# zouyuoz/SVS-UNet-PyTorch

Hardware: AMD Instinct MI355X
Metric: spectrogram-tiles/sec (512x128) U-Net fwd+bwd (L1 train step incl. Adam) (higher is better)
Workload: dtype f32; 1 GPU; train.py L1-loss step, 512x128 tiles, batch 64 per GPU; global_batch=64, parallelism=dp1, mode=train

## Files before the change

### include/svs_hip.h

```cpp
#ifndef SVS_HIP_H
#define SVS_HIP_H

#include <stddef.h>
#include <stdint.h>

typedef struct ihipStream_t* hipStream_t;

#ifdef __cplusplus
extern "C" {
#endif

#define SVS_OK 0
#define SVS_ERR_INVALID (-1)
#define SVS_ERR_WORKSPACE (-2)
#define SVS_ABI_VERSION 1

int svs_version(void);
const char* svs_last_error_string(void);
int svs_tuning_set(const char* name, long value);

int svs_fill_uniform(float* out, int64_t n, uint32_t seed, uint64_t offset, float scale, float shift,
                     hipStream_t stream);
int svs_fill_tiles(float* mix, float* voc, int B, int H, int W, int64_t first_tile, hipStream_t stream);
int svs_crop_tiles(const float* mix_songs, const float* voc_songs, const int64_t* offset, const int32_t* frames,
// ... 49 lines not shown
int svs_bn_act_apply(const float* raw, int64_t ldr, int64_t P, int C, int64_t pixels_per_sample,
                     const float* gamma, const float* beta, const float* save_mean, const float* save_invstd,
                     float slope, const float* drop, float* y, int64_t ldy, hipStream_t stream);
int svs_bn_bwd(const float* dy, int64_t lddy, const float* raw, int64_t ldr, int64_t P, int C,
               int64_t pixels_per_sample, const float* gamma, const float* beta,
               const float* save_mean, const float* save_invstd, float slope, const float* drop,
               float* d_raw, float* dgamma, float* dbeta, void* ws, size_t ws_bytes, hipStream_t stream);

size_t svs_l1_mask_loss_workspace_bytes(int64_t n);
int svs_l1_mask_loss_fwd_bwd(const float* mask, const float* mix, const float* voc, int64_t n, float loss_scale,
                             float* d_logit, float* loss, void* ws, size_t ws_bytes, hipStream_t stream);

int svs_adam_step(float* p, const float* g, float* m, float* v, int64_t n, double lr, double beta1, double beta2,
                  double eps, int step, float grad_scale, hipStream_t stream);

int svs_apply_mask(const float* mix, const float* mask, float* out, int64_t n, int invert, hipStream_t stream);

#define SVS_UNET_NUM_PARAMS 46
#define SVS_UNET_NUM_BN 11
int64_t svs_unet_param_offset(int tensor_index);
int64_t svs_unet_buffer_offset(int bn_index, int which );

size_t svs_unet_prepared_bytes(void);
int svs_unet_prepare_eval(const float* params, const float* bn_buffers, void* prepared, hipStream_t stream);
size_t svs_unet_eval_workspace_bytes(int B, int H, int W);
int svs_unet_forward_eval(const void* prepared, const float* mix, float* mask, int B, int H, int W,
                          void* ws, size_t ws_bytes, hipStream_t stream);

size_t svs_unet_train_workspace_bytes(int B, int H, int W);
int svs_unet_train_fwd_bwd(const float* params, float* grads, float* bn_buffers, int64_t* num_batches_tracked,
                           const float* mix, const float* voc, const float* drop, int B, int H, int W,
                           float loss_scale, float* mask , float* loss,
                           void* ws, size_t ws_bytes, hipStream_t stream);
int svs_unet_train_forward(const float* params, float* bn_buffers, int64_t* num_batches_tracked,
                           const float* mix, const float* drop, int B, int H, int W, float* mask,
                           void* ws, size_t ws_bytes, hipStream_t stream);
int svs_unet_train_backward(const float* params, float* grads, const float* mix, const float* mask,
                            const float* d_mask, const float* drop, int B, int H, int W,
                            void* ws, size_t ws_bytes, hipStream_t stream);
int svs_unet_train_fwd_loss(const float* params, float* bn_buffers, int64_t* num_batches_tracked, const float* mix,
                            const float* voc, const float* drop, int B, int H, int W, float loss_scale,
                            float* mask , float* loss, void* ws, size_t ws_bytes, hipStream_t stream);
int svs_unet_train_bwd_part(const float* params, float* grads, const float* mix, const float* drop, int B, int H, int W,
                            int part, void* ws, size_t ws_bytes, hipStream_t stream);
int svs_unet_train_bwd_sync(hipStream_t consumer);
size_t svs_unet_train_mr_workspace_bytes(int B, int W, int hop);
int svs_unet_train_fwd_loss_mr(const float* params, float* bn_buffers, int64_t* num_batches_tracked, const float* mix,
                               const float* voc, const float* mix_phase, const float* voc_phase, const float* drop, int B, int H,
                               int W, int hop, float alpha_l1, float alpha_mr, float* mask, float* losses, void* ws, size_t ws_bytes,
                               void* mr_ws, size_t mr_ws_bytes, hipStream_t stream);
int64_t svs_unet_ws_offset(const char* name, int B, int H, int W, int training);

size_t svs_unet_prepared_bf16_bytes(void);
int svs_unet_prepare_eval_bf16(const void* prepared_f32, void* prepared_bf16, hipStream_t stream);
size_t svs_unet_eval_bf16_workspace_bytes(int B, int H, int W);
int svs_unet_forward_eval_bf16(const void* prepared_bf16, const float* mix, float* mask, int B, int H, int W, void* ws,
                               size_t ws_bytes, hipStream_t stream);

int svs_stft_frames(int64_t n_samples, int hop);
int svs_stft_fwd(const float* y, int64_t n_samples, int n_fft, int hop, float* mag, float* phase,
                 hipStream_t stream);
size_t svs_istft_workspace_bytes(int n_fft, int hop, int frames);
int svs_istft(const float* mag, const float* phase, int phase_is_angle, int n_fft, int hop, int frames,
              float* y, void* ws, size_t ws_bytes, hipStream_t stream);
int svs_stft_tiles(const float* y, int64_t n_samples, int channels, int n_fft, int hop, float* mag, int64_t chan_stride,
                   int seg, int rows, int first_bin, int frames_alloc, float* phase, int phase_mode,
// ... 50 lines not shown
```

### svs_unet_pytorch_amd/_lib.py

```python
from __future__ import annotations

import ctypes as C
import os
import re

HERE = os.path.dirname(os.path.abspath(__file__))
LIB_PATH = os.environ.get("SVS_LIB_PATH") or os.path.join(HERE, "libsvs_hip.so")
HEADER_PATH = os.path.join(os.path.dirname(HERE), "include", "svs_hip.h")

_lib = None

P = C.c_void_p
I = C.c_int
L = C.c_int64
F = C.c_float
D = C.c_double
Z = C.c_size_t
U32 = C.c_uint32
U64 = C.c_uint64

_SIGS = {
    "svs_version": (I, []),
    "svs_last_error_string": (C.c_char_p, []),
    "svs_tuning_set": (I, [C.c_char_p, C.c_long]),
    "svs_fill_uniform": (I, [P, L, U32, U64, F, F, P]),
    "svs_fill_tiles": (I, [P, P, I, I, I, L, P]),
    "svs_crop_tiles": (I, [P, P, P, P, P, P, I, I, I, P, P, P]),
    "svs_phase_angle": (I, [P, P, L, P]),
    "svs_dropout_mask": (I, [P, I, I, I, U32, I, I, P]),
    "svs_dropout_masks_all": (I, [P, I, U32, I, I, P]),
    "svs_pack_weight_gather": (I, [P, P, I, I, P]),
    "svs_pack_weight_parity": (I, [P, P, I, I, P]),
    "svs_bn_fold": (I, [P, P, P, P, P, F, P, P, I, P]),
    "svs_enc_block_workspace_bytes": (Z, [I, I, I, I, I]),
    "svs_enc_block_fwd": (I, [P, L, I, I, I, I, P, P, P, P, F, P, L, I, I, P, Z, P]),
    "svs_dec_block_workspace_bytes": (Z, [I, I, I, I, I, I, I]),
    "svs_dec_block_fwd": (I, [P, L, I, I, I, I, P, P, P, P, F, P, L, I, I, I, I, P, Z, P]),
    "svs_out_block_fwd": (I, [P, L, I, I, I, I, P, P, P, I, I, I, P]),
    "svs_enc_block_bwd_data": (I, [P, L, I, I, I, I, P, P, L, I, I, I, I, P, Z, P]),
    "svs_dec_block_bwd_data": (I, [P, L, I, I, I, I, P, P, L, I, I, I, I, P, Z, P]),
    "svs_block_bwd_weight_workspace_bytes": (Z, [I, I, I, I, I]),
    "svs_enc_block_bwd_weight": (I, [P, L, I, I, I, I, P, L, I, I, I, P, P, P, Z, P]),
    "svs_dec_block_bwd_weight": (I, [P, L, I, I, I, I, P, L, I, I, I, P, P, P, Z, P]),
    "svs_describe_plan": (I, [I, I, I, I, I, I, I, I, C.c_char_p, Z]),
    "svs_bn_workspace_bytes": (Z, [L, I]),
    "svs_bn_stats": (I, [P, L, L, I, P, Z, P]),
    "svs_bn_finalize": (I, [P, L, I, F, F, P, P, P, P, P, P]),
    "svs_bn_act_apply": (I, [P, L, L, I, L, P, P, P, P, F, P, P, L, P]),
    "svs_bn_bwd": (I, [P, L, P, L, L, I, L, P, P, P, P, F, P, P, P, P, P, Z, P]),
    "svs_l1_mask_loss_workspace_bytes": (Z, [L]),
    "svs_l1_mask_loss_fwd_bwd": (I, [P, P, P, L, F, P, P, P, Z, P]),
    "svs_adam_step": (I, [P, P, P, P, L, D, D, D, D, I, F, P]),
    "svs_apply_mask": (I, [P, P, P, L, I, P]),
    "svs_unet_param_offset": (L, [I]),
    "svs_unet_buffer_offset": (L, [I, I]),
    "svs_unet_prepared_bytes": (Z, []),
    "svs_unet_prepare_eval": (I, [P, P, P, P]),
    "svs_unet_eval_workspace_bytes": (Z, [I, I, I]),
    "svs_unet_forward_eval": (I, [P, P, P, I, I, I, P, Z, P]),
    "svs_unet_prepared_bf16_bytes": (Z, []),
    "svs_unet_prepare_eval_bf16": (I, [P, P, P]),
    "svs_unet_eval_bf16_workspace_bytes": (Z, [I, I, I]),
    "svs_unet_forward_eval_bf16": (I, [P, P, P, I, I, I, P, Z, P]),
    "svs_unet_train_workspace_bytes": (Z, [I, I, I]),
    "svs_unet_train_fwd_bwd": (I, [P, P, P, P, P, P, P, I, I, I, F, P, P, P, Z, P]),
    "svs_unet_train_forward": (I, [P, P, P, P, P, I, I, I, P, P, Z, P]),
    "svs_unet_train_backward": (I, [P, P, P, P, P, P, I, I, I, P, Z, P]),
    "svs_unet_train_fwd_loss": (I, [P, P, P, P, P, P, I, I, I, F, P, P, P, Z, P]),
    "svs_unet_train_bwd_part": (I, [P, P, P, P, I, I, I, I, P, Z, P]),
    "svs_unet_train_bwd_sync": (I, [P]),
    "svs_unet_train_mr_workspace_bytes": (Z, [I, I, I]),
    "svs_unet_train_fwd_loss_mr": (I, [P, P, P, P, P, P, P, P, I, I, I, I, F, F, P, P, P, Z, P, Z, P]),
    "svs_unet_ws_offset": (L, [C.c_char_p, I, I, I, I]),
    "svs_stft_frames": (I, [L, I]),
    "svs_stft_fwd": (I, [P, L, I, I, P, P, P]),
    "svs_istft_workspace_bytes": (Z, [I, I, I]),
    "svs_istft": (I, [P, P, I, I, I, I, P, P, Z, P]),
    "svs_stft_tiles": (I, [P, L, I, I, I, P, L, I, I, I, I, P, I, P, P]),
    "svs_stft_groups": (I, [I]),
    "svs_istft_tiles": (I, [P, L, I, I, I, P, I, P, I, I, I, I, I, P, P, P]),
    "svs_istft_groups": (I, [I, I, I]),
    "svs_transpose_c64": (I, [P, P, I, I, P]),
    "svs_istft_bwd_mask": (I, [P, P, P, P, P, F, I, I, I, I, P]),
    "svs_mrstft_workspace_bytes": (Z, [I, L]),
    "svs_mrstft_loss_fwd_bwd": (I, [P, P, I, L, F, P, P, P, Z, P]),
    "svs_absmax": (I, [P, L, P, P, Z, P]),
    "svs_max": (I, [P, L, P, P]),
    "svs_scale_by_inv": (I, [P, L, P, F, P]),
    "svs_bss_corr_workspace_bytes": (Z, [L, I, P]),
    "svs_bss_corr": (I, [P, L, I, L, P, I, P, P, Z, P]),
    "svs_bss_solve_workspace_bytes": (Z, [I, I, I]),
    "svs_bss_solve": (I, [P, I, I, P, P, I, P, P, P, Z, P]),
    "svs_bss_corr_windows_workspace_bytes": (Z, [L, L, I, P]),
    "svs_bss_corr_windows": (I, [P, L, I, L, L, L, L, P, I, P, L, P, Z, P]),
    "svs_bss_solve_batched_workspace_bytes": (Z, [L, I, I, I]),
    "svs_bss_solve_batched": (I, [P, L, I, I, P, P, I, P, P, P, Z, P]),
    "svs_resample_out_len": (L, [L, I, I]),
    "svs_resample_table_bytes": (Z, [I, I, I]),
# ... 50 lines not shown
```

### svs_unet_pytorch_amd/csrc/elementwise.hip

```cpp
#include "unet_desc.h"

static inline int red_blocks(long P, int C) {
  long nb = (P * C) / 4096;
  if (nb > 1024) nb = 1024;
  if (nb < 1) nb = 1;
  return (int)nb;
}

struct RedPlan { int sw, nslab, lp, rows; long ppr; };
static RedPlan red_plan(long P, int C) {
  RedPlan r;
  r.sw = C < 32 ? C : 32;
  r.nslab = C / r.sw;
  r.lp = r.sw / 4;
  long nb = (P * C) / 4096;
  if (nb > 512) nb = 512;
  long rows = nb / r.nslab;
  if (rows < 1) rows = 1;
  r.ppr = (P + rows - 1) / rows;
  r.rows = (int)((P + r.ppr - 1) / r.ppr);
  return r;
}
static inline int red_rows(long P, int C) { return red_plan(P, C).rows; }

// ... 593 lines not shown
}
extern "C" int svs_scale_by_inv(float* x, int64_t n, const float* denom, float numer, hipStream_t stream) {
  SVS_REQUIRE(x && denom && n > 0, "svs_scale_by_inv: null pointer");
  hipLaunchKernelGGL(scale_by_inv_kernel, dim3(grid_for(n)), dim3(256), 0, stream, x, (long)n, denom, numer);
  SVS_CHECK_LAUNCH("scale_by_inv");
  return SVS_OK;
}

__global__ __launch_bounds__(256) void adam_kernel(float* __restrict__ p, const float* __restrict__ g, float* __restrict__ m,
                                                   float* __restrict__ v, long n, float b1, float b2, float omb1,
                                                   float omb2, float eps, float step_size, float bc2_sqrt, float gscale) {
  for (long i = (long)blockIdx.x * 256 + threadIdx.x; i < n; i += (long)gridDim.x * 256) {
    const float gi = g[i] * gscale;
    const float mi = m[i] * b1 + omb1 * gi;
    const float vi = v[i] * b2 + omb2 * gi * gi;
    m[i] = mi;
    v[i] = vi;
    const float denom = sqrtf(vi) / bc2_sqrt + eps;
    p[i] -= step_size * (mi / denom);
  }
}
extern "C" int svs_adam_step(float* p, const float* g, float* m, float* v, int64_t n, double lr, double beta1, double beta2,
                             double eps, int step, float grad_scale, hipStream_t stream) {
  SVS_REQUIRE(p && g && m && v && n > 0 && step >= 1, "svs_adam_step: bad arguments");
  const double bc1 = 1.0 - pow(beta1, step);
  const double bc2 = 1.0 - pow(beta2, step);
  hipLaunchKernelGGL(adam_kernel, dim3(grid_for(n)), dim3(256), 0, stream, p, g, m, v, (long)n, (float)beta1,
                     (float)beta2, (float)(1.0 - beta1), (float)(1.0 - beta2), (float)eps, (float)(lr / bc1), (float)sqrt(bc2),
                     grad_scale);
  SVS_CHECK_LAUNCH("adam");
  return SVS_OK;
}

__global__ __launch_bounds__(256) void apply_mask_kernel(const float* __restrict__ mix, const float* __restrict__ mask,
                                                         float* __restrict__ out, long n, int invert) {
  for (long i = (long)blockIdx.x * 256 + threadIdx.x; i < n; i += (long)gridDim.x * 256) {
    float m = mask[i];
    if (invert) m = 1.f - m;
    out[i] = mix[i] * m;
  }
}
extern "C" int svs_apply_mask(const float* mix, const float* mask, float* out, int64_t n, int invert, hipStream_t stream) {
  SVS_REQUIRE(mix && mask && out && n > 0, "svs_apply_mask: null pointer");
  hipLaunchKernelGGL(apply_mask_kernel, dim3(grid_for(n)), dim3(256), 0, stream, mix, mask, out, (long)n, invert);
  SVS_CHECK_LAUNCH("apply_mask");
  return SVS_OK;
}

__global__ __launch_bounds__(256) void pack_gather_kernel(const float* __restrict__ w, float* __restrict__ wp, int N, int C) {
  const long total = (long)N * C * 25;
  for (long o = (long)blockIdx.x * 256 + threadIdx.x; o < total; o += (long)gridDim.x * 256) {
    const int c = (int)(o % C);
    const long r = o / C;
    const int tap = (int)(r % 25);
    const long n = r / 25;
    wp[o] = w[(n * C + c) * 25 + tap];
  }
}
extern "C" int svs_pack_weight_gather(const float* w, float* wp, int N, int C, hipStream_t stream) {
  SVS_REQUIRE(w && wp && N > 0 && C > 0, "svs_pack_weight_gather: bad arguments");
  hipLaunchKernelGGL(pack_gather_kernel, dim3(grid_for((long)N * C * 25)), dim3(256), 0, stream, w, wp, N, C);
  SVS_CHECK_LAUNCH("pack_gather");
  return SVS_OK;
}

__global__ __launch_bounds__(256) void pack_parity_kernel(const float* __restrict__ w, float* __restrict__ wp, int C, int N) {
// ... 44 lines not shown
    for (int e = threadIdx.x; e < tot; e += 256) {
      const int c = e / 25, tap = e - c * 25;
      tile[e] = jb.w[((long)c * N + n) * 25 + tap];
    }
    __syncthreads();
    const long NC = (long)N * C;
#pragma unroll
    for (int par = 0; par < 4; ++par) {
      const int ph = par >> 1, pw = par & 1, ntw = 3 - pw, ntaps = (3 - ph) * ntw;
      const int poff = (par == 0) ? 0 : (par == 1) ? 9 : (par == 2) ? 15 : 21;
      float* dst = jb.wp + poff * NC + (long)n * ntaps * C;
      for (int e = threadIdx.x; e < ntaps * C; e += 256) {
        const int t2 = lc >= 0 ? e >> lc : e / C, c = e - t2 * C;
        const int th = t2 / ntw, tw = t2 - th * ntw;
        dst[e] = tile[c * 25 + (ph + 2 * th) * 5 + pw + 2 * tw];
      }
    }
  }
}

int svs_pack_all_run(SvsPackJobs& jobs, hipStream_t stream) {
  int blocks = 0;
  for (int i = 0; i < jobs.n; ++i) {
    SVS_REQUIRE(jobs.j[i].C <= 512 && jobs.j[i].w && jobs.j[i].wp, "svs_pack_all: bad job %d", i);
    jobs.j[i].first_block = blocks;
    blocks += jobs.j[i].N;
  }
  if (!blocks) return SVS_OK;
  hipLaunchKernelGGL(pack_all_kernel, dim3(blocks), dim3(256), 0, stream, jobs);
  SVS_CHECK_LAUNCH("pack_all");
  return SVS_OK;
}

__global__ void bn_fold_kernel(const float* gamma, const float* beta, const float* rm, const float* rv, const float* bias,
                               float eps, float* scale, float* shift, int C) {
  const int c = blockIdx.x * blockDim.x + threadIdx.x;
  if (c >= C) return;
  const float s = gamma[c] / sqrtf(rv[c] + eps);
  scale[c] = s;
  shift[c] = beta[c] + ((bias ? bias[c] : 0.f) - rm[c]) * s;
}
extern "C" int svs_bn_fold(const float* gamma, const float* beta, const float* running_mean, const float* running_var,
                           const float* conv_bias, float eps, float* scale, float* shift, int C, hipStream_t stream) {
  SVS_REQUIRE(gamma && beta && running_mean && running_var && scale && shift && C > 0, "svs_bn_fold: bad arguments");
  hipLaunchKernelGGL(bn_fold_kernel, dim3((C + 63) / 64), dim3(64), 0, stream, gamma, beta, running_mean, running_var,
                     conv_bias, eps, scale, shift, C);
  SVS_CHECK_LAUNCH("bn_fold");
  return SVS_OK;
}

__global__ __launch_bounds__(256) void fill_uniform_kernel(float* out, long n, uint32_t seed, uint64_t offset, float scale, float shift) {
  for (long i = (long)blockIdx.x * 256 + threadIdx.x; i < n; i += (long)gridDim.x * 256)
    out[i] = (float)(svs_u32(seed, offset + (uint64_t)i) >> 8) * 5.9604644775390625e-08f * scale + shift;
}
extern "C" int svs_fill_uniform(float* out, int64_t n, uint32_t seed, uint64_t offset, float scale, float shift, hipStream_t stream) {
  SVS_REQUIRE(out && n > 0, "svs_fill_uniform: bad arguments");
  hipLaunchKernelGGL(fill_uniform_kernel, dim3(grid_for(n)), dim3(256), 0, stream, out, (long)n, seed, offset, scale, shift);
  SVS_CHECK_LAUNCH("fill_uniform");
  return SVS_OK;
}

__global__ __launch_bounds__(256) void fill_tiles_kernel(float* mix, float* voc, long per, long total, long first_tile) {
  for (long i = (long)blockIdx.x * 256 + threadIdx.x; i < total; i += (long)gridDim.x * 256) {
    const long b = i / per;
    const uint64_t ctr = (uint64_t)(i - b * per) + ((uint64_t)(first_tile + b) << 32);
    const float m = (float)(svs_u32(0u, ctr) >> 8) * 5.9604644775390625e-08f;
// ... 87 lines not shown
```

### svs_unet_pytorch_amd/csrc/internal.h

```cpp
#pragma once
#include "common.h"

enum { SVS_MODE_GATHER = 0, SVS_MODE_PARITY = 1 };

int svs_conv_gemm_run(int mode, const float* x, long ldx, int B, int H, int W, int C, const float* wp,
                      const float* bias, const float* scale, const float* shift, float slope, float* y, long ldy,
                      int Ho, int Wo, int N, int accumulate, void* ws, size_t ws_bytes, hipStream_t stream,
                      const char* who, float* stats = nullptr, int stats_cap = 0, int* stats_nblk = nullptr);
int svs_bn_finalize_run(const void* partial, int nblk, long P, int C, float eps, float momentum, float* running_mean,
                        float* running_var, long long* nbt, float* save_mean, float* save_invstd, hipStream_t stream);
int svs_bn_fin_act_apply_run(const void* partial, int rows, const float* raw, long ldr, long P, int C, long pixels_per_sample,
                             const float* gamma, const float* beta, float eps, float momentum, float* running_mean,
                             float* running_var, long long* nbt, float* save_mean, float* save_invstd, float slope,
                             const float* drop, float* y, long ldy, hipStream_t stream);
struct SvsSumJobs { int njobs; const float* partial[12]; int nblk[12]; int C[12]; float* out[12]; };
int svs_channel_sum_finalize_multi_run(const SvsSumJobs& jobs, hipStream_t stream);
size_t svs_bn_partial_floats(long P, int C);
int svs_bn_partial_rows(long P, int C);
size_t svs_conv_gemm_workspace(int mode, int B, int H, int W, int C, int Ho, int Wo, int N);

int svs_wgrad_gemm_run(const float* s, long lds, int B, int Hs, int Ws, int Cs, const float* l, long ldl, int Hl,
                       int Wl, int Cl, float* dw, void* ws, size_t ws_bytes, hipStream_t stream, const char* who);
size_t svs_wgrad_gemm_workspace(int B, int Hs, int Ws, int Cs, int Cl);

int svs_conv_c1_run(const float* x, int B, int H, int W, const float* w, const float* bias, const float* scale,
                    const float* shift, float slope, float* y, long ldy, int N, int accumulate, hipStream_t stream,
                    const char* who, long half = 0);
int svs_deconv_to1_run(const float* x, long ldx, int B, int H, int W, int C, const float* w, const float* bias,
                       float* y, int Ho, int Wo, int apply_sigmoid, hipStream_t stream, const char* who, long half = 0);
int svs_wgrad_c1_run(const float* s, long lds, int B, int Hs, int Ws, int Cs, const float* l, int Hl, int Wl,
                     float* dw, void* ws, size_t ws_bytes, hipStream_t stream, const char* who, long half = 0);
size_t svs_wgrad_c1_workspace(int B, int Hs, int Ws, int Cs);

int svs_channel_sum_run(const float* x, long ldx, long P, int C, float* out, void* ws, size_t ws_bytes, hipStream_t stream);
int svs_sum_run(const float* x, long n, float* out, void* ws, size_t ws_bytes, hipStream_t stream);
int svs_sigmoid_bwd_run(const float* mask, const float* dmask, long n, float* d_logit, hipStream_t stream);

int svs_reduce_slabs_run(const float* slab, int nslab, int per, int groups, long n, float* out, hipStream_t stream);

struct SvsPackJob { const float* w; float* wp; int N, C, kind, first_block; };
struct SvsPackJobs { SvsPackJob j[20]; int n; };
int svs_pack_all_run(SvsPackJobs& jobs, hipStream_t stream);

int svs_bn_bwd_run(const float* dy, long lddy, const float* raw, long ldr, long P, int C, long pixels_per_sample,
                   const float* gamma, const float* beta, const float* save_mean, const float* save_invstd, float slope,
                   const float* drop, float* d_raw, float* dgamma, float* dbeta, float* dbias, void* ws, size_t ws_bytes,
                   hipStream_t stream, float* dbias_partial = nullptr, SvsSumJobs* defer = nullptr);

int svs_fft_twiddles(int n, hipStream_t stream, const float2** out);

int svs_conv_gemm_describe(int mode, int B, int H, int W, int C, int Ho, int Wo, int N, long ldx, char* buf, size_t n);
int svs_wgrad_gemm_describe(int B, int Hs, int Ws, int Cs, int Cl, char* buf, size_t n);
```

### svs_unet_pytorch_amd/csrc/net.hip

```cpp
#include <math.h>
#include <algorithm>
#include <atomic>
#include <mutex>
#include <stdarg.h>
#include <stdlib.h>
#include <string.h>

#include "unet_desc.h"

static thread_local char g_err[512] = "";
void svs_set_error(const char* fmt, ...) {
  va_list ap;
  va_start(ap, fmt);
  vsnprintf(g_err, sizeof(g_err), fmt, ap);
  va_end(ap);
}
extern "C" const char* svs_last_error_string(void) { return g_err; }

static const char* const TUNE_NAMES[SVS_TUNE_COUNT] = {
    "CONV_CFG", "CONV_KSPLIT", "CONV_WINDOW", "CONV_SKIP", "SKIP_REDUCE", "WGRAD_CFG", "WGRAD_KSPLIT", "WGRAD_SKIP",
    "WGRAD_WINDOW", "TRAIN_UNFUSED", "TRAIN_ONE_STREAM", "MFMA_SPLIT", "CONV_C1_TILED", "BF16_CFG", "BF16_KSPLIT", "BN_INLINE",
    "CONV_GWINDOW"};
static std::atomic<long> g_tune[SVS_TUNE_COUNT];
static std::once_flag g_tune_once;
// ... 293 lines not shown
  }
  return g_side[dev];
}

extern "C" size_t svs_unet_train_workspace_bytes(int B, int H, int W) {
  Geo g;
  if (make_geo(B, H, W, g)) return 0;
  return train_layout(g, nullptr).total;
}

struct WsName { const char* stem; int first, count; float* const* p; };
static int64_t ws_find(const WsName* tab, size_t n, const char* name, const char* base) {
  for (size_t i = 0; i < n; ++i) {
    const size_t len = strlen(tab[i].stem);
    if (strncmp(name, tab[i].stem, len)) continue;
    if (!tab[i].count) {
      if (!name[len]) return (const char*)*tab[i].p - base;
      continue;
    }
    char* end;
    const long idx = strtol(name + len, &end, 10) - tab[i].first;
    if (end != name + len && !*end && idx >= 0 && idx < tab[i].count) return (const char*)tab[i].p[idx] - base;
  }
  return -1;
}
extern "C" int64_t svs_unet_ws_offset(const char* name, int B, int H, int W, int training) {
  Geo g;
  if (!name || make_geo(B, H, W, g)) return -1;
  char* const base = (char*)256;
  if (training) {
    const TrainWs t = train_layout(g, base);
    const WsName tab[] = {{"cat", 1, 5, t.cat + 1}, {"c6", 0, 0, &t.c6},         {"raw_e", 1, 6, t.raw},  {"raw_d", 1, 5, t.raw + 6},
                          {"dcat", 1, 5, t.dcat + 1}, {"dc6", 0, 0, &t.dc6},     {"d_logit", 0, 0, &t.d_logit}, {"mask", 0, 0, &t.mask},
                          {"mean", 0, 11, t.mean},  {"invstd", 0, 11, t.invstd}};
    return ws_find(tab, sizeof(tab) / sizeof(tab[0]), name, base);
  }
  const EvalWs e = eval_layout(g, base);
  const WsName tab[] = {{"cat", 1, 5, e.cat + 1}, {"c6", 0, 0, &e.c6}};
  return ws_find(tab, sizeof(tab) / sizeof(tab[0]), name, base);
}

struct TrainCall { Geo g; TrainWs t; ParamView v; };
static int train_prologue(const char* who, const float* params, int B, int H, int W, void* ws, size_t ws_bytes, TrainCall& c) {
  const int rc = make_geo(B, H, W, c.g);
  if (rc) return rc;
  c.t = train_layout(c.g, ws);
  if (!ws || ws_bytes < c.t.total || !svs_aligned16(ws)) {
    svs_set_error("%s: workspace too small (%zu < %zu)", who, ws_bytes, c.t.total);
    return SVS_ERR_WORKSPACE;
  }
  c.v = view_params(params);
  return SVS_OK;
}

static int train_bn_act(const TrainCall& c, int l, int stat_rows, float* bn_buffers, int64_t* nbt, float slope, const float* drop,
                        View y, hipStream_t stream) {
  const TrainWs& t = c.t;
  const int N = bn_channels(l), lvl = bn_level(l);
  const long P = c.g.P[lvl];
  if (!stat_rows) {
    const int rc = svs_bn_stats(t.raw[l], N, P, N, t.bnws, t.bnws_bytes, stream);
    if (rc) return rc;
    stat_rows = svs_bn_partial_rows(P, N);
  }
  return svs_bn_fin_act_apply_run(t.bnws, stat_rows, t.raw[l], N, P, N, (long)c.g.h[lvl] * c.g.w[lvl], c.v.gamma[l], c.v.beta[l], BN_EPS,
                                  BN_MOMENTUM, bn_buffers ? bn_buffers + svs_unet_buffer_offset(l, 0) : nullptr,
                                  bn_buffers ? bn_buffers + svs_unet_buffer_offset(l, 1) : nullptr,
                                  nbt ? (long long*)(nbt + l) : nullptr, t.mean[l], t.invstd[l], slope, drop, y.p, y.ld, stream);
}

static int train_forward_impl(const TrainCall& c, float* bn_buffers, int64_t* nbt, const float* mix, const float* drop, float* mask,
                              hipStream_t stream) {
  const Geo& g = c.g; const TrainWs& t = c.t; const ParamView& v = c.v;
  const int B = g.B;
  int rc;
  const int fused_rows = svs_tune_flag(SVS_TUNE_TRAIN_UNFUSED) ? 0 : (int)(t.bnws_bytes / sizeof(float));
  SideStream* sd = svs_tune_flag(SVS_TUNE_TRAIN_ONE_STREAM) ? nullptr : side_stream(stream);
  std::unique_lock<std::mutex> guard;
  if (sd) guard = std::unique_lock<std::mutex>(sd->mu);
  {
    SvsPackJobs jobs{};
    for (int l = 1; l <= 10; ++l) {
      const Layer& L = LAYERS[l];
      jobs.j[jobs.n++] = SvsPackJob{v.w[l], t.wfwd[l], L.N, L.C, L.up, 0};
      jobs.j[jobs.n++] = SvsPackJob{v.w[l], t.wbwd[l], L.C, L.N, !L.up, 0};
    }
    if (sd) {
      SVS_HIP(hipEventRecord(sd->fork[0], stream));
      SVS_HIP(hipStreamWaitEvent(sd->s, sd->fork[0], 0));
    }
    if ((rc = svs_pack_all_run(jobs, sd ? sd->s : stream))) return rc;
    if (sd) SVS_HIP(hipEventRecord(sd->done[0], sd->s));
  }
  for (int k = 1; k <= 6; ++k) {
    if (k == 2 && sd) SVS_HIP(hipStreamWaitEvent(stream, sd->done[0], 0));
    const int l = k - 1;
    const View xi = (k == 1) ? View{const_cast<float*>(mix), 1} : cat_half(t.cat, g, k - 1, 1);
    int stat_rows = 0;
    if (k == 1) rc = svs_enc_block_fwd(xi.p, xi.ld, B, g.h[0], g.w[0], 1, v.w[0], v.b[0], nullptr, nullptr, 0.f, t.raw[0], CH[1], CH[1], 0,
                                       t.scratch, t.scratch_bytes, stream);
    else rc = svs_conv_gemm_run(SVS_MODE_GATHER, xi.p, xi.ld, B, g.h[k - 1], g.w[k - 1], CH[k - 1], t.wfwd[l], v.b[l], nullptr, nullptr, 0.f,
                                t.raw[l], CH[k], g.h[k], g.w[k], CH[k], 0, t.scratch, t.scratch_bytes, stream, "conv forward",
                                t.bnws, fused_rows, &stat_rows);
    if (rc) return rc;
    const View yo = (k == 6) ? View{t.c6, CH[6]} : cat_half(t.cat, g, k, 1);
    if ((rc = train_bn_act(c, l, stat_rows, bn_buffers, nbt, LEAKY, nullptr, yo, stream))) return rc;
  }
  const float* dp = drop;
  for (int l = 6; l <= 10; ++l) {
    const Layer& D = LAYERS[l];
    const float* x = (l == 6) ? t.c6 : t.cat[D.lin];
    int stat_rows = 0;
    rc = svs_conv_gemm_run(SVS_MODE_PARITY, x, D.C, B, g.h[D.lin], g.w[D.lin], D.C, t.wfwd[l], v.b[l], nullptr, nullptr, 0.f,
                           t.raw[l], D.N, g.h[D.lout], g.w[D.lout], D.N, 0, t.scratch, t.scratch_bytes, stream,
                           "deconv forward", t.bnws, fused_rows, &stat_rows);
    if (rc) return rc;
    if ((rc = train_bn_act(c, l, stat_rows, bn_buffers, nbt, 0.f, dp, cat_half(t.cat, g, D.lout, 0), stream))) return rc;
    if (dp) dp += (long)B * D.N;
  }
  return svs_deconv_to1_run(t.cat[1], CH[1], B, g.h[1], g.w[1], LAYERS[11].C, v.w[11], v.b[11], mask, g.h[0], g.w[0], 1, stream,
                            "svs_unet_train_forward", level1_plane(g));
}

static int train_backward_impl(const TrainCall& c, float* grads, const float* mix, const float* drop, hipStream_t stream, int parts = 15) {
  const Geo& g = c.g; const TrainWs& t = c.t; const ParamView& v = c.v;
  const int B = g.B;
  int rc;
  auto G = [&](int idx) { return grads + svs_unet_param_offset(idx); };
  SvsSumJobs sums{};
  const bool unfused = svs_tune_flag(SVS_TUNE_TRAIN_UNFUSED);
  SideStream* sd = svs_tune_flag(SVS_TUNE_TRAIN_ONE_STREAM) ? nullptr : side_stream(stream);
  std::unique_lock<std::mutex> guard;
  if (sd) guard = std::unique_lock<std::mutex>(sd->mu);
  const hipStream_t wstream = sd ? sd->s : stream;
  float* const wscratch = sd ? t.scratch2 : t.scratch;
  const size_t wscratch_bytes = sd ? t.scratch2_bytes : t.scratch_bytes;
  int nfork_local = 0;
  int& nfork = sd ? sd->nfork : nfork_local;
  if (parts & 1) nfork = 0;
  auto layer_draw = [&](int l) -> float* { return sd ? t.d_raw_l[l] : t.d_raw; };
  auto fork = [&]() -> int {
    if (!sd) return SVS_OK;
    SVS_HIP(hipEventRecord(sd->fork[nfork & 3], stream));
    SVS_HIP(hipStreamWaitEvent(sd->s, sd->fork[nfork & 3], 0));
    return SVS_OK;
  };
  auto forked = [&]() -> int { ++nfork; return SVS_OK; };
  auto join = [&]() -> int {
    if (sd && nfork > 0) {
      SVS_HIP(hipEventRecord(sd->done[0], sd->s));
      SVS_HIP(hipStreamWaitEvent(stream, sd->done[0], 0));
    }
    return SVS_OK;
  };
  if (parts & 1) {
  const long half1 = level1_plane(g);
  if ((rc = fork())) return rc;
  if ((rc = svs_wgrad_c1_run(t.cat[1], CH[1], B, g.h[1], g.w[1], LAYERS[11].C, t.d_logit, g.h[0], g.w[0], G(44), wscratch, wscratch_bytes, wstream,
                             "deconv6 bwd_weight", half1))) return rc;
  if ((rc = svs_sum_run(t.d_logit, g.P[0], G(45), wscratch, wscratch_bytes, wstream))) return rc;
  if ((rc = forked())) return rc;
  if ((rc = svs_conv_c1_run(t.d_logit, B, g.h[0], g.w[0], v.w[11], nullptr, nullptr, nullptr, 0.f, t.dcat[1], CH[1], LAYERS[11].C, 0, stream,
                            "deconv6 bwd_data", half1))) return rc;
  long drop_off[11];
  { long o = 0; for (int l = 6; l <= 10; ++l) { drop_off[l] = o; o += (long)B * LAYERS[l].N; } }
  for (int l = 10; l >= 6; --l) {
    const int lin = LAYERS[l].lin, lout = LAYERS[l].lout, N = LAYERS[l].N, C = LAYERS[l].C;
    const float* x = (l == 6) ? t.c6 : t.cat[lin];
    const View dyv = cat_half(t.dcat, g, lout, 0);
    float* const d_raw = layer_draw(l);
    rc = svs_bn_bwd_run(dyv.p, dyv.ld, t.raw[l], N, g.P[lout], N, (long)g.h[lout] * g.w[lout], v.gamma[l], v.beta[l],
                        t.mean[l], t.invstd[l], 0.f, drop ? drop + drop_off[l] : nullptr, d_raw, G(4 * l + 2), G(4 * l + 3),
                        G(4 * l + 1), t.bnws, t.bnws_bytes, stream, unfused ? nullptr : t.dbias_part[l], &sums);
    if (rc) return rc;
    if ((rc = fork())) return rc;
    if ((rc = svs_dec_block_bwd_weight(x, C, B, g.h[lin], g.w[lin], C, d_raw, N, g.h[lout], g.w[lout], N, G(4 * l), nullptr,
                                       wscratch, wscratch_bytes, wstream))) return rc;
    if ((rc = forked())) return rc;
    float* dx = (l == 6) ? t.dc6 : t.dcat[lin];
    if ((rc = svs_dec_block_bwd_data(d_raw, N, B, g.h[lout], g.w[lout], N, t.wbwd[l], dx, C, g.h[lin], g.w[lin], C, 0,
                                     t.scratch, t.scratch_bytes, stream))) return rc;
  }
  if ((rc = svs_channel_sum_finalize_multi_run(sums, stream))) return rc;
  sums.njobs = 0;
  }
  if (!(parts & 14)) return SVS_OK;
  for (int k = 6; k >= 1; --k) {
    if (!(parts & (k == 6 ? 2 : k >= 4 ? 4 : 8))) continue;
    const int l = k - 1, N = CH[k], C = CH[k - 1];
    const View dyv = (k == 6) ? View{t.dc6, CH[6]} : cat_half(t.dcat, g, k, 1);
    float* const d_raw = layer_draw(l);
    rc = svs_bn_bwd_run(dyv.p, dyv.ld, t.raw[l], N, g.P[k], N, (long)g.h[k] * g.w[k], v.gamma[l], v.beta[l], t.mean[l], t.invstd[l],
                        LEAKY, nullptr, d_raw, G(4 * l + 2), G(4 * l + 3), G(4 * l + 1), t.bnws, t.bnws_bytes, stream,
                        unfused ? nullptr : t.dbias_part[l], &sums);
    if (rc) return rc;
    const View xi = (k == 1) ? View{const_cast<float*>(mix), 1} : cat_half(t.cat, g, k - 1, 1);
    const float* x = xi.p; const long ldx = xi.ld;
    if (k == 1) {
      if ((rc = svs_enc_block_bwd_weight(d_raw, N, B, g.h[k], g.w[k], N, x, ldx, g.h[k - 1], g.w[k - 1], C, G(4 * l), nullptr,
                                         t.scratch, t.scratch_bytes, stream))) return rc;
      continue;
    }
    if ((rc = fork())) return rc;
    if ((rc = svs_enc_block_bwd_weight(d_raw, N, B, g.h[k], g.w[k], N, x, ldx, g.h[k - 1], g.w[k - 1], C, G(4 * l), nullptr,
                                       wscratch, wscratch_bytes, wstream))) return rc;
    if ((rc = forked())) return rc;
    if (k >= 2) {
      const View dxs = cat_half(t.dcat, g, k - 1, 1);
      if ((rc = svs_enc_block_bwd_data(d_raw, N, B, g.h[k], g.w[k], N, t.wbwd[l], dxs.p, dxs.ld, g.h[k - 1], g.w[k - 1], C, 1,
                                       t.scratch, t.scratch_bytes, stream))) return rc;
    }
  }
  if ((rc = svs_channel_sum_finalize_multi_run(sums, stream))) return rc;
  return (parts & 8) ? join() : SVS_OK;
}

extern "C" int svs_unet_train_bwd_sync(hipStream_t consumer) {
  SideStream* sd = svs_tune_flag(SVS_TUNE_TRAIN_ONE_STREAM) ? nullptr : side_stream(consumer);
  if (!sd) return SVS_OK;
  std::lock_guard<std::mutex> guard(sd->mu);
  SVS_HIP(hipEventRecord(sd->sync, sd->s));
  SVS_HIP(hipStreamWaitEvent(consumer, sd->sync, 0));
  return SVS_OK;
}

extern "C" int svs_unet_train_forward(const float* params, float* bn_buffers, int64_t* num_batches_tracked, const float* mix,
                                      const float* drop, int B, int H, int W, float* mask, void* ws, size_t ws_bytes,
                                      hipStream_t stream) {
  SVS_REQUIRE(params && mix && mask && svs_aligned16(params) && svs_aligned16(mix) && svs_aligned16(mask), "svs_unet_train_forward: bad pointers");
  TrainCall c;
  const int rc = train_prologue("svs_unet_train_forward", params, B, H, W, ws, ws_bytes, c);
  if (rc) return rc;
  return train_forward_impl(c, bn_buffers, num_batches_tracked, mix, drop, mask, stream);
}

extern "C" int svs_unet_train_backward(const float* params, float* grads, const float* mix, const float* mask,
                                       const float* d_mask, const float* drop, int B, int H, int W, void* ws,
                                       size_t ws_bytes, hipStream_t stream) {
  SVS_REQUIRE(params && grads && mix && mask && d_mask && svs_aligned16(grads), "svs_unet_train_backward: bad pointers");
  TrainCall c;
  int rc = train_prologue("svs_unet_train_backward", params, B, H, W, ws, ws_bytes, c);
  if (rc) return rc;
  if ((rc = svs_sigmoid_bwd_run(mask, d_mask, c.g.P[0], c.t.d_logit, stream))) return rc;
  return train_backward_impl(c, grads, mix, drop, stream);
}

static int train_fwd_loss_impl(const TrainCall& c, float* bn_buffers, int64_t* nbt, const float* mix, const float* voc, const float* drop,
                               float loss_scale, float* mask, float* loss, hipStream_t stream) {
  float* m = mask ? mask : c.t.mask;
  const int rc = train_forward_impl(c, bn_buffers, nbt, mix, drop, m, stream);
  if (rc) return rc;
  return svs_l1_mask_loss_fwd_bwd(m, mix, voc, c.g.P[0], loss_scale, c.t.d_logit, loss, c.t.bnws, c.t.bnws_bytes, stream);
}

extern "C" int svs_unet_train_fwd_bwd(const float* params, float* grads, float* bn_buffers, int64_t* num_batches_tracked,
                                      const float* mix, const float* voc, const float* drop, int B, int H, int W,
                                      float loss_scale, float* mask, float* loss, void* ws, size_t ws_bytes,
                                      hipStream_t stream) {
  SVS_REQUIRE(params && grads && mix && voc && loss && svs_aligned16(params) && svs_aligned16(grads) && svs_aligned16(mix),
              "svs_unet_train_fwd_bwd: bad pointers");
  TrainCall c;
  int rc = train_prologue("svs_unet_train_fwd_bwd", params, B, H, W, ws, ws_bytes, c);
  if (rc) return rc;
  if ((rc = train_fwd_loss_impl(c, bn_buffers, num_batches_tracked, mix, voc, drop, loss_scale, mask, loss, stream))) return rc;
  return train_backward_impl(c, grads, mix, drop, stream);
}

extern "C" int svs_unet_train_fwd_loss(const float* params, float* bn_buffers, int64_t* num_batches_tracked, const float* mix,
                                       const float* voc, const float* drop, int B, int H, int W, float loss_scale, float* mask,
                                       float* loss, void* ws, size_t ws_bytes, hipStream_t stream) {
  SVS_REQUIRE(params && mix && voc && loss && svs_aligned16(params) && svs_aligned16(mix), "svs_unet_train_fwd_loss: bad pointers");
  TrainCall c;
  const int rc = train_prologue("svs_unet_train_fwd_loss", params, B, H, W, ws, ws_bytes, c);
  if (rc) return rc;
  return train_fwd_loss_impl(c, bn_buffers, num_batches_tracked, mix, voc, drop, loss_scale, mask, loss, stream);
}

struct MrTrainWs { float* wav_pred; float* wav_tgt; float* d_wav; void* mr; size_t mr_bytes; size_t total; };
static MrTrainWs mr_train_layout(int B, int W, int hop, void* ws) {
  MrTrainWs m{};
  Arena a{(char*)ws, 0};
  const size_t L = (size_t)hop * (W - 1);
  m.wav_pred = a.take<float>((size_t)B * L);
  m.wav_tgt = a.take<float>((size_t)B * L);
  m.d_wav = a.take<float>((size_t)B * L);
  m.mr_bytes = svs_mrstft_workspace_bytes(B, (int64_t)L);
  m.mr = a.take<float>(m.mr_bytes / sizeof(float) + 64);
  m.total = a.used;
  return m;
}
extern "C" size_t svs_unet_train_mr_workspace_bytes(int B, int W, int hop) {
  if (B <= 0 || W < 2 || hop <= 0) return 0;
  return mr_train_layout(B, W, hop, nullptr).total;
}
extern "C" int svs_unet_train_fwd_loss_mr(const float* params, float* bn_buffers, int64_t* num_batches_tracked, const float* mix,
                                          const float* voc, const float* mix_phase, const float* voc_phase, const float* drop,
                                          int B, int H, int W, int hop, float alpha_l1, float alpha_mr, float* mask, float* losses,
                                          void* ws, size_t ws_bytes, void* mr_ws, size_t mr_ws_bytes, hipStream_t stream) {
// ... 28 lines not shown
```

### svs_unet_pytorch_amd/model.py

```python
from __future__ import annotations

import os

import numpy as np
import torch
import torch.nn as nn

from . import _lib
from ._lib import check, lib, ptr
from .synth import DEC_IO, ENC_CHANNELS


def _on_model_device(fn):
    import functools

    @functools.wraps(fn)
    def wrapped(self, *a, **k):
        dev = (self._model if hasattr(self, "_model") else self)._flat.device
        if dev.type != "cuda" or torch.cuda.current_device() == dev.index:
            return fn(self, *a, **k)
        with torch.cuda.device(dev):
            return fn(self, *a, **k)
    return wrapped

ALPHA_L1 = 166.66
ALPHA_MR = 0.66


class WeightedL1Loss(nn.Module):

    def __init__(self, reduction="mean"):
        super().__init__()
        self.reduction = reduction

    @staticmethod
# ... 106 lines not shown
    def __init__(self):
        super().__init__()
        for k in range(6):
            cin, cout = ENC_CHANNELS[k], ENC_CHANNELS[k + 1]
            setattr(self, f"conv{k + 1}", nn.Sequential(
                nn.Conv2d(cin, cout, kernel_size=(5, 5), stride=(2, 2), padding=2),
                nn.BatchNorm2d(cout),
                nn.LeakyReLU(negative_slope=0.2, inplace=True)))
        for j, (cin, cout) in enumerate(DEC_IO):
            setattr(self, f"deconv{j + 1}", nn.ConvTranspose2d(cin, cout, kernel_size=(5, 5), stride=(2, 2), padding=2))
            if j < 5:
                setattr(self, f"deconv{j + 1}_BAD", nn.Sequential(nn.BatchNorm2d(cout), nn.ReLU(True), nn.Dropout2d(0.5)))

        self.loss_list_vocal = []
        self.loss_list_accomp = []
        self.loss_list_total = []

        self._param_list = list(self.parameters())
        self._param_spans = []
        off = 0
        for p in self._param_list:
            self._param_spans.append((off, p.numel()))
            off += p.numel()
        self._n_params = off
        self._bn_list = [getattr(self, f"conv{k + 1}")[1] for k in range(6)] + \
                        [getattr(self, f"deconv{j + 1}_BAD")[0] for j in range(5)]
        self._flat = self._gflat = self._bn_flat = self._nbt_flat = None
        self._param_epoch = 0
        self._prepared = None
        self._prepared_key = None
        self._ws = {}
        self._generation = 0
        self._grads_clean = True
        self._anchor = None
        self._injected_masks = None
        self.dropout_seed = 4242
        self._xstream = None
        self.dropout_step = 0
        self.last_mr_loss = None
        self.eval_precision = "fp32"
        self._prepared_bf16 = None
        self._prepared_bf16_key = None
        self.rank = 0
        self._flatten()

        self.optim = FusedAdam(self, lr=1e-3)
        self.crit = nn.L1Loss()

    def _flatten(self):
        dev = self._param_list[0].device
        with torch.no_grad():
            flat = torch.empty(self._n_params, dtype=torch.float32, device=dev)
            gflat = torch.zeros(self._n_params, dtype=torch.float32, device=dev)
            for p, (off, n) in zip(self._param_list, self._param_spans):
                flat[off:off + n].copy_(p.data.reshape(-1).to(torch.float32))
                p.data = flat[off:off + n].view(p.shape)
                p.grad = gflat[off:off + n].view(p.shape)
            nbn = sum(2 * bn.num_features for bn in self._bn_list)
            bn_flat = torch.empty(nbn, dtype=torch.float32, device=dev)
            nbt = torch.empty(len(self._bn_list), dtype=torch.int64, device=dev)
            off = 0
            for i, bn in enumerate(self._bn_list):
                c = bn.num_features
                bn_flat[off:off + c].copy_(bn.running_mean)
                bn_flat[off + c:off + 2 * c].copy_(bn.running_var)
                nbt[i] = bn.num_batches_tracked
                bn.running_mean = bn_flat[off:off + c]
                bn.running_var = bn_flat[off + c:off + 2 * c]
                bn.num_batches_tracked = nbt[i]
                off += 2 * c
        self._flat, self._gflat, self._bn_flat, self._nbt_flat = flat, gflat, bn_flat, nbt
        self._prepared = None
        self._prepared_key = None
        self._ws = {}
        self._anchor = torch.zeros(1, device=dev, requires_grad=True)
        self._param_epoch += 1
        if hasattr(self, "optim"):
            self.optim._ensure_state()

    def _apply(self, fn, recurse=True):
        out = super()._apply(fn, recurse)
        self._flatten()
        return out

    def _attach_grads(self):
        for p, (off, n) in zip(self._param_list, self._param_spans):
            g = p.grad
            if g is None or g.data_ptr() != self._gflat.data_ptr() + 4 * off:
                p.grad = self._gflat[off:off + n].view(p.shape)

    def load(self, path):
        if os.path.exists(path):
            print("Load the pre-trained model from {}".format(path))
            state = torch.load(path, map_location="cpu")
            for key, obj in state.items():
                if "loss_list" in key:
                    setattr(self, key, obj)
            self.load_state_dict(state["model_state_dict"], strict=False)
            if "optim" in state:
                self.optim.load_state_dict(state["optim"])
            self.dropout_step = int(state.get("dropout_step", self.optim._step))
        else:
            print("Pre-trained model {} is not exist...".format(path))

    def save(self, path):
        state = {"model_state_dict": self.state_dict(), "optim": self.optim.state_dict(), "dropout_step": self.dropout_step}
        for key in self.__dict__:
# ... 208 lines not shown

    @_on_model_device
    def fwd_bwd_overlapped(self, mix, voc, loss_scale, grad_sync, mix_phase=None, voc_phase=None, alpha_mr=0.0):
        mix, voc = self._check_input(mix), self._check_input(voc)
        B, _, H, W = mix.shape
        ws = self._workspace("train", B, H, W)
        self._drop = self._drop_masks(B)
        self._generation += 1
        self._param_epoch += 1
        self._attach_grads()
        assert self._grads_clean, "overlapped exchange needs zero_grad() first (it overwrites the flat gradient buffer)"
        L = lib()
        loss = self._fwd_losses(mix, voc, loss_scale, mix_phase, voc_phase, alpha_mr, ws)
        split = int(L.svs_unet_param_offset(24))
        c6 = int(L.svs_unet_param_offset(20))
        c4 = int(L.svs_unet_param_offset(12))
        handles = []
        main = torch.cuda.current_stream(mix.device)
        if self._xstream is None:
            self._xstream = torch.cuda.Stream(device=mix.device)
        xs = self._xstream
        for part, sl in ((0, self._gflat[split:]), (2, self._gflat[c6:split]), (5, self._gflat[c4:c6]), (6, self._gflat[:c4])):
            check(L.svs_unet_train_bwd_part(ptr(self._flat), ptr(self._gflat), ptr(mix), ptr(self._drop), B, H, W, part, ptr(ws),
                                            ws.numel(), _lib.stream_ptr()), "svs_unet_train_bwd_part")
            xs.wait_stream(main)
            check(L.svs_unet_train_bwd_sync(xs.cuda_stream), "svs_unet_train_bwd_sync")
            with torch.cuda.stream(xs):
                handles.append(grad_sync.reduce_async(sl))
        self._grads_clean = False
        return loss, handles

    def train_step(self, mix, voc, loss_scale=1.0, grad_sync=None, mix_phase=None, voc_phase=None, alpha_mr=0.0):
        self.optim.zero_grad()
        if grad_sync is not None and getattr(grad_sync, "overlap", False):
            loss, handles = self.fwd_bwd_overlapped(mix, voc, loss_scale, grad_sync, mix_phase, voc_phase, alpha_mr)
            for h in handles:
                h.wait()
        else:
            loss = self.fwd_bwd(mix, voc, loss_scale, mix_phase, voc_phase, alpha_mr)
            if grad_sync is not None:
                grad_sync(self._gflat)
        self.optim.step()
        return loss

    def backward(self, mix, voc):
        loss = self.train_step(mix, voc)
        self.loss_list_total.append(loss.item())
```

Baseline: 19030 tiles/s.

## Fuse Adam update and weight repacking into the backward pass per layer group

Adds a single train-step entry that runs forward, loss, backward and the Adam update in one call. Adam updates for each layer group are issued on the weight-gradient stream as soon as that group's gradients finish, and the packed forward/backward weight layouts are rebuilt right there. On the next step the forward pass can skip repacking when the Python side confirms the packings are still current. This is meant to overlap the optimiser and packing with the rest of backward and to cut launch and host overhead, at the cost of extra bookkeeping that could go stale if parameters change outside the tracked versions.

```diff
diff --git a/include/svs_hip.h b/include/svs_hip.h
--- a/include/svs_hip.h
+++ b/include/svs_hip.h
@@ -105,6 +105,16 @@
                            const float* mix, const float* voc, const float* drop, int B, int H, int W,
                            float loss_scale, float* mask , float* loss,
                            void* ws, size_t ws_bytes, hipStream_t stream);
+typedef struct SvsAdamDesc {
+  float* m; float* v;
+  double lr, beta1, beta2, eps;
+  int step;
+  float grad_scale;
+} SvsAdamDesc;
+int svs_unet_train_step(float* params, float* grads, float* bn_buffers, int64_t* num_batches_tracked,
+                        const float* mix, const float* voc, const float* drop, int B, int H, int W,
+                        float loss_scale, float* mask , float* loss, const SvsAdamDesc* opt,
+                        int packings_current, void* ws, size_t ws_bytes, hipStream_t stream);
 int svs_unet_train_forward(const float* params, float* bn_buffers, int64_t* num_batches_tracked,
                            const float* mix, const float* drop, int B, int H, int W, float* mask,
                            void* ws, size_t ws_bytes, hipStream_t stream);
diff --git a/svs_unet_pytorch_amd/_lib.py b/svs_unet_pytorch_amd/_lib.py
--- a/svs_unet_pytorch_amd/_lib.py
+++ b/svs_unet_pytorch_amd/_lib.py
@@ -18,6 +18,11 @@
 Z = C.c_size_t
 U32 = C.c_uint32
 U64 = C.c_uint64
+
+
+class AdamDesc(C.Structure):
+    _fields_ = [("m", P), ("v", P), ("lr", D), ("beta1", D), ("beta2", D), ("eps", D), ("step", I), ("grad_scale", F)]
+
 
 _SIGS = {
     "svs_version": (I, []),
@@ -64,6 +69,7 @@
     "svs_unet_forward_eval_bf16": (I, [P, P, P, I, I, I, P, Z, P]),
     "svs_unet_train_workspace_bytes": (Z, [I, I, I]),
     "svs_unet_train_fwd_bwd": (I, [P, P, P, P, P, P, P, I, I, I, F, P, P, P, Z, P]),
+    "svs_unet_train_step": (I, [P, P, P, P, P, P, P, I, I, I, F, P, P, C.POINTER(AdamDesc), I, P, Z, P]),
     "svs_unet_train_forward": (I, [P, P, P, P, P, I, I, I, P, P, Z, P]),
     "svs_unet_train_backward": (I, [P, P, P, P, P, P, I, I, I, P, Z, P]),
     "svs_unet_train_fwd_loss": (I, [P, P, P, P, P, P, I, I, I, F, P, P, P, Z, P]),
diff --git a/svs_unet_pytorch_amd/csrc/elementwise.hip b/svs_unet_pytorch_amd/csrc/elementwise.hip
--- a/svs_unet_pytorch_amd/csrc/elementwise.hip
+++ b/svs_unet_pytorch_amd/csrc/elementwise.hip
@@ -649,6 +649,17 @@
   return SVS_OK;
 }
 
+int svs_adam_range_run(const SvsAdamDesc& a, float* p, const float* g, long first, long n, hipStream_t stream) {
+  SVS_REQUIRE(p && g && a.m && a.v && first >= 0 && n > 0 && a.step >= 1, "svs_adam_range: bad arguments");
+  const double bc1 = 1.0 - pow(a.beta1, a.step);
+  const double bc2 = 1.0 - pow(a.beta2, a.step);
+  hipLaunchKernelGGL(adam_kernel, dim3(grid_for(n)), dim3(256), 0, stream, p + first, g + first, a.m + first, a.v + first, n,
+                     (float)a.beta1, (float)a.beta2, (float)(1.0 - a.beta1), (float)(1.0 - a.beta2), (float)a.eps,
+                     (float)(a.lr / bc1), (float)sqrt(bc2), a.grad_scale);
+  SVS_CHECK_LAUNCH("adam");
+  return SVS_OK;
+}
+
 __global__ __launch_bounds__(256) void apply_mask_kernel(const float* __restrict__ mix, const float* __restrict__ mask,
                                                          float* __restrict__ out, long n, int invert) {
   for (long i = (long)blockIdx.x * 256 + threadIdx.x; i < n; i += (long)gridDim.x * 256) {
@@ -759,6 +770,13 @@
   return SVS_OK;
 }
 
+int svs_pack_range_run(const SvsPackJobs& all, int first, int count, hipStream_t stream) {
+  SVS_REQUIRE(first >= 0 && count >= 0 && first + count <= all.n, "svs_pack_range: bad range %d+%d of %d", first, count, all.n);
+  SvsPackJobs piece{};
+  for (int i = 0; i < count; ++i) piece.j[piece.n++] = all.j[first + i];
+  return svs_pack_all_run(piece, stream);
+}
+
 __global__ void bn_fold_kernel(const float* gamma, const float* beta, const float* rm, const float* rv, const float* bias,
                                float eps, float* scale, float* shift, int C) {
   const int c = blockIdx.x * blockDim.x + threadIdx.x;
diff --git a/svs_unet_pytorch_amd/csrc/internal.h b/svs_unet_pytorch_amd/csrc/internal.h
--- a/svs_unet_pytorch_amd/csrc/internal.h
+++ b/svs_unet_pytorch_amd/csrc/internal.h
@@ -41,6 +41,9 @@
 struct SvsPackJob { const float* w; float* wp; int N, C, kind, first_block; };
 struct SvsPackJobs { SvsPackJob j[20]; int n; };
 int svs_pack_all_run(SvsPackJobs& jobs, hipStream_t stream);
+int svs_pack_range_run(const SvsPackJobs& all, int first, int count, hipStream_t stream);
+
+int svs_adam_range_run(const SvsAdamDesc& a, float* p, const float* g, long first, long n, hipStream_t stream);
 
 int svs_bn_bwd_run(const float* dy, long lddy, const float* raw, long ldr, long P, int C, long pixels_per_sample,
                    const float* gamma, const float* beta, const float* save_mean, const float* save_invstd, float slope,
diff --git a/svs_unet_pytorch_amd/csrc/net.hip b/svs_unet_pytorch_amd/csrc/net.hip
--- a/svs_unet_pytorch_amd/csrc/net.hip
+++ b/svs_unet_pytorch_amd/csrc/net.hip
@@ -349,7 +349,7 @@
     const TrainWs t = train_layout(g, base);
     const WsName tab[] = {{"cat", 1, 5, t.cat + 1}, {"c6", 0, 0, &t.c6},         {"raw_e", 1, 6, t.raw},  {"raw_d", 1, 5, t.raw + 6},
                           {"dcat", 1, 5, t.dcat + 1}, {"dc6", 0, 0, &t.dc6},     {"d_logit", 0, 0, &t.d_logit}, {"mask", 0, 0, &t.mask},
-                          {"mean", 0, 11, t.mean},  {"invstd", 0, 11, t.invstd}};
+                          {"mean", 0, 11, t.mean},  {"invstd", 0, 11, t.invstd},   {"wfwd", 1, 10, t.wfwd + 1},   {"wbwd", 1, 10, t.wbwd + 1}};
     return ws_find(tab, sizeof(tab) / sizeof(tab[0]), name, base);
   }
   const EvalWs e = eval_layout(g, base);
@@ -386,8 +386,14 @@
                                   nbt ? (long long*)(nbt + l) : nullptr, t.mean[l], t.invstd[l], slope, drop, y.p, y.ld, stream);
 }
 
+static void add_pack_jobs(const TrainCall& c, int l, SvsPackJobs& jobs) {
+  const Layer& L = LAYERS[l];
+  jobs.j[jobs.n++] = SvsPackJob{c.v.w[l], c.t.wfwd[l], L.N, L.C, L.up, 0};
+  jobs.j[jobs.n++] = SvsPackJob{c.v.w[l], c.t.wbwd[l], L.C, L.N, !L.up, 0};
+}
+
 static int train_forward_impl(const TrainCall& c, float* bn_buffers, int64_t* nbt, const float* mix, const float* drop, float* mask,
-                              hipStream_t stream) {
+                              hipStream_t stream, bool packed = false) {
   const Geo& g = c.g; const TrainWs& t = c.t; const ParamView& v = c.v;
   const int B = g.B;
   int rc;
@@ -395,13 +401,10 @@
   SideStream* sd = svs_tune_flag(SVS_TUNE_TRAIN_ONE_STREAM) ? nullptr : side_stream(stream);
   std::unique_lock<std::mutex> guard;
   if (sd) guard = std::unique_lock<std::mutex>(sd->mu);
-  {
+  const bool join_pack = sd && !packed;
+  if (!packed) {
     SvsPackJobs jobs{};
-    for (int l = 1; l <= 10; ++l) {
-      const Layer& L = LAYERS[l];
-      jobs.j[jobs.n++] = SvsPackJob{v.w[l], t.wfwd[l], L.N, L.C, L.up, 0};
-      jobs.j[jobs.n++] = SvsPackJob{v.w[l], t.wbwd[l], L.C, L.N, !L.up, 0};
-    }
+    for (int l = 1; l <= 10; ++l) add_pack_jobs(c, l, jobs);
     if (sd) {
       SVS_HIP(hipEventRecord(sd->fork[0], stream));
       SVS_HIP(hipStreamWaitEvent(sd->s, sd->fork[0], 0));
@@ -410,7 +413,7 @@
     if (sd) SVS_HIP(hipEventRecord(sd->done[0], sd->s));
   }
   for (int k = 1; k <= 6; ++k) {
-    if (k == 2 && sd) SVS_HIP(hipStreamWaitEvent(stream, sd->done[0], 0));
+    if (k == 2 && join_pack) SVS_HIP(hipStreamWaitEvent(stream, sd->done[0], 0));
     const int l = k - 1;
     const View xi = (k == 1) ? View{const_cast<float*>(mix), 1} : cat_half(t.cat, g, k - 1, 1);
     int stat_rows = 0;
@@ -439,7 +442,9 @@
                             "svs_unet_train_forward", level1_plane(g));
 }
 
-static int train_backward_impl(const TrainCall& c, float* grads, const float* mix, const float* drop, hipStream_t stream, int parts = 15) {
+static int train_backward_impl(const TrainCall& c, float* grads, const float* mix, const float* drop, hipStream_t stream, int parts = 15,
+                               const SvsAdamDesc* opt = nullptr, float* opt_params = nullptr) {
+  SVS_REQUIRE(!opt || (parts == 15 && opt_params), "train_backward: the optimiser runs inside a whole backward pass only");
   const Geo& g = c.g; const TrainWs& t = c.t; const ParamView& v = c.v;
   const int B = g.B;
   int rc;
@@ -470,6 +475,14 @@
     }
     return SVS_OK;
   };
+  auto update = [&](int t0, int t1, int l0, int l1, hipStream_t s) -> int {
+    if (!opt) return SVS_OK;
+    const long first = svs_unet_param_offset(t0);
+    if ((rc = svs_adam_range_run(*opt, opt_params, grads, first, svs_unet_param_offset(t1) - first, s))) return rc;
+    SvsPackJobs jobs{};
+    for (int l = l0; l <= l1; ++l) add_pack_jobs(c, l, jobs);
+    return svs_pack_range_run(jobs, 0, jobs.n, s);
+  };
   if (parts & 1) {
   const long half1 = level1_plane(g);
   if ((rc = fork())) return rc;
@@ -522,14 +535,23 @@
     if ((rc = svs_enc_block_bwd_weight(d_raw, N, B, g.h[k], g.w[k], N, x, ldx, g.h[k - 1], g.w[k - 1], C, G(4 * l), nullptr,
                                        wscratch, wscratch_bytes, wstream))) return rc;
     if ((rc = forked())) return rc;
+    if (k == 6 && (rc = update(24, SVS_UNET_NUM_PARAMS, 6, 10, wstream))) return rc;
+    if (k == 5 && (rc = update(20, 24, 5, 5, wstream))) return rc;
+    if (k == 3 && (rc = update(12, 20, 3, 4, wstream))) return rc;
     if (k >= 2) {
       const View dxs = cat_half(t.dcat, g, k - 1, 1);
       if ((rc = svs_enc_block_bwd_data(d_raw, N, B, g.h[k], g.w[k], N, t.wbwd[l], dxs.p, dxs.ld, g.h[k - 1], g.w[k - 1], C, 1,
                                        t.scratch, t.scratch_bytes, stream))) return rc;
     }
+    if (opt && (k == 6 || k == 4)) {
+      if ((rc = svs_channel_sum_finalize_multi_run(sums, stream))) return rc;
+      sums.njobs = 0;
+    }
   }
   if ((rc = svs_channel_sum_finalize_multi_run(sums, stream))) return rc;
-  return (parts & 8) ? join() : SVS_OK;
+  if (!(parts & 8)) return SVS_OK;
+  if ((rc = join())) return rc;
+  return update(0, 12, 1, 2, stream);
 }
 
 extern "C" int svs_unet_train_bwd_sync(hipStream_t consumer) {
@@ -563,9 +585,9 @@
 }
 
 static int train_fwd_loss_impl(const TrainCall& c, float* bn_buffers, int64_t* nbt, const float* mix, const float* voc, const float* drop,
-                               float loss_scale, float* mask, float* loss, hipStream_t stream) {
+                               float loss_scale, float* mask, float* loss, hipStream_t stream, bool packed = false) {
   float* m = mask ? mask : c.t.mask;
-  const int rc = train_forward_impl(c, bn_buffers, nbt, mix, drop, m, stream);
+  const int rc = train_forward_impl(c, bn_buffers, nbt, mix, drop, m, stream, packed);
   if (rc) return rc;
   return svs_l1_mask_loss_fwd_bwd(m, mix, voc, c.g.P[0], loss_scale, c.t.d_logit, loss, c.t.bnws, c.t.bnws_bytes, stream);
 }
@@ -581,6 +603,20 @@
   if (rc) return rc;
   if ((rc = train_fwd_loss_impl(c, bn_buffers, num_batches_tracked, mix, voc, drop, loss_scale, mask, loss, stream))) return rc;
   return train_backward_impl(c, grads, mix, drop, stream);
+}
+
+extern "C" int svs_unet_train_step(float* params, float* grads, float* bn_buffers, int64_t* num_batches_tracked,
+                                   const float* mix, const float* voc, const float* drop, int B, int H, int W,
+                                   float loss_scale, float* mask, float* loss, const SvsAdamDesc* opt, int packings_current,
+                                   void* ws, size_t ws_bytes, hipStream_t stream) {
+  SVS_REQUIRE(params && grads && mix && voc && loss && svs_aligned16(params) && svs_aligned16(grads) && svs_aligned16(mix),
+              "svs_unet_train_step: bad pointers");
+  SVS_REQUIRE(opt && opt->m && opt->v && opt->step >= 1, "svs_unet_train_step: bad optimiser description");
+  TrainCall c;
+  int rc = train_prologue("svs_unet_train_step", params, B, H, W, ws, ws_bytes, c);
+  if (rc) return rc;
+  if ((rc = train_fwd_loss_impl(c, bn_buffers, num_batches_tracked, mix, voc, drop, loss_scale, mask, loss, stream, packings_current != 0))) return rc;
+  return train_backward_impl(c, grads, mix, drop, stream, 15, opt, params);
 }
 
 extern "C" int svs_unet_train_fwd_loss(const float* params, float* bn_buffers, int64_t* num_batches_tracked, const float* mix,
diff --git a/svs_unet_pytorch_amd/model.py b/svs_unet_pytorch_amd/model.py
--- a/svs_unet_pytorch_amd/model.py
+++ b/svs_unet_pytorch_amd/model.py
@@ -1,6 +1,8 @@
 from __future__ import annotations
 
+import ctypes
 import os
+import weakref
 
 import numpy as np
 import torch
@@ -173,6 +175,7 @@
         self._ws = {}
         self._generation = 0
         self._grads_clean = True
+        self._packed = None
         self._anchor = None
         self._injected_masks = None
         self.dropout_seed = 4242
@@ -214,6 +217,7 @@
         self._prepared = None
         self._prepared_key = None
         self._ws = {}
+        self._packed = None
         self._anchor = torch.zeros(1, device=dev, requires_grad=True)
         self._param_epoch += 1
         if hasattr(self, "optim"):
@@ -488,6 +492,8 @@
 
     def train_step(self, mix, voc, loss_scale=1.0, grad_sync=None, mix_phase=None, voc_phase=None, alpha_mr=0.0):
         self.optim.zero_grad()
+        if grad_sync is None and (mix_phase is None or not alpha_mr):
+            return self._fused_step(mix, voc, loss_scale)
         if grad_sync is not None and getattr(grad_sync, "overlap", False):
             loss, handles = self.fwd_bwd_overlapped(mix, voc, loss_scale, grad_sync, mix_phase, voc_phase, alpha_mr)
             for h in handles:
@@ -499,6 +505,40 @@
         self.optim.step()
         return loss
 
+    def _pack_key(self):
+        return (self._flat.data_ptr(), self._flat._version, self._param_epoch, sum(p._version for p in self._param_list))
+
+    def _packings_current(self, ws):
+        packed = self._packed
+        return packed is not None and packed[0]() is ws and packed[1] == self._pack_key()
+
+    @_on_model_device
+    def _fused_step(self, mix, voc, loss_scale):
+        mix, voc = self._check_input(mix), self._check_input(voc)
+        B, _, H, W = mix.shape
+        ws = self._workspace("train", B, H, W)
+        current = self._packings_current(ws)
+        self._packed = None
+        self._drop = self._drop_masks(B)
+        self._generation += 1
+        self._param_epoch += 1
+        self._attach_grads()
+        self.last_mr_loss = None
+        opt = self.optim
+        opt._ensure_state()
+        g = opt.param_groups[0]
+        opt._step += 1
+        desc = _lib.AdamDesc(ptr(opt._m), ptr(opt._v), float(g["lr"]), float(g["betas"][0]), float(g["betas"][1]), float(g["eps"]),
+                             int(opt._step), float(opt.grad_scale))
+        loss = torch.empty(1, dtype=torch.float32, device=mix.device)
+        check(lib().svs_unet_train_step(ptr(self._flat), ptr(self._gflat), ptr(self._bn_flat), ptr(self._nbt_flat), ptr(mix), ptr(voc),
+                                        ptr(self._drop), B, H, W, float(loss_scale), None, ptr(loss), ctypes.byref(desc), int(current),
+                                        ptr(ws), ws.numel(), _lib.stream_ptr()), "svs_unet_train_step")
+        self._grads_clean = False
+        self._param_epoch += 1
+        self._packed = (weakref.ref(ws), self._pack_key())
+        return loss[0]
+
     def backward(self, mix, voc):
         loss = self.train_step(mix, voc)
         self.loss_list_total.append(loss.item())
```

Measured after the change: 18780 tiles/s. 1.3% lower.
